# LikeLy-Journey/SegmenTron

Measured on AMD Instinct MI355X. Metric: images/sec fwd+bwd DeepLabv3+_xception65 @1025x2049, higher is better.
Workload: dtype bf16; 1 GPU; DeepLabv3+_xception65 train step (fwd + CE loss + bwd + SGD) @1025x2049, batch 2/GPU (BASELINE.json configs[2]); global_batch=2, bn=BN, parallelism=dp1, full_size=True

## Files before the change

### include/segmentron_hip.h

```cpp
#ifndef SEGMENTRON_HIP_H
#define SEGMENTRON_HIP_H
#ifdef __cplusplus
extern "C" {
#endif

const char* seg_last_error(void);
int seg_version(void);

int seg_conv_gemm_fwd(int dtype, const void* x, long ldx, int N, int Hi, int Wi, int C,
                      const void* w, int O, int KH, int KW, int stride, int pad, int dil,
                      int pro_mode, const float* pro_scale, const float* pro_shift,
                      const float* bias, void* y, long ldy, int Ho, int Wo, int out_H, int out_W,
                      int out_s, float* stat_partial, const void* ep_x, long ldep,
                      const float* ep_c0, const float* ep_c1, int tconv, void* stream);
int seg_conv_gemm_tiles_m(int N, int Ho, int Wo);

int seg_conv_gemm_wgrad(int dtype, const void* x, long ldx, int N, int Hi, int Wi, int C,
                        const void* dy, long lddy, int Ho, int Wo, int O, int KH, int KW,
                        int stride, int pad, int dil, int pro_mode, const float* pro_scale,
                        const float* pro_shift, float* partial, int splits, void* stream);
int seg_conv_gemm_stat_rows(int dtype, int N, int Ho, int Wo, int C, int O, int KH, int KW,
                            int stride, int pad, int dil, int tconv, int has_bias, int pro_mode);
int seg_conv_gemm_wgrad_splits(int dtype, int N, int Ho, int Wo, int C, int O, int KH, int KW,
                               int stride, int pad, int dil, int pro_mode);

int seg_dwconv3x3(int dtype, int mode, const void* x, long ldx, int N, int Hi, int Wi, int C,
                  const float* w9c, int w_layout, int stride, int dil, int pro_mode,
                  const float* pro_scale, const float* pro_shift, void* y, long ldy, int Ho, int Wo,
                  float* stat_partial, int grid_y, void* stream);
int seg_dwconv_grid_y(int dtype, int C, int N, int Ho, int Wo, int stride, int dil, int kind);
int seg_dwconv3x3_wgrad_finalize(const float* partial, int R, int C, float* dw_c9, void* stream);
int seg_dwconv3x3_wgrad(int dtype, const void* x, long ldx, int N, int Hi, int Wi, int C,
                        const void* dy, long lddy, int Ho, int Wo, int stride, int dil,
                        int pro_mode, const float* pro_scale, const float* pro_shift,
                        float* partial, int grid_y, void* stream);

int seg_dwconv3x3_bwd_fused(int dtype, const void* dy, long lddy, const void* x, long ldx, int N,
                            int H, int W, int C, const float* w9c, int w_layout, int dil,
                            int pro_mode, const float* pro_scale, const float* pro_shift, void* g,
                            long ldg, float* partial_w, float* partial_bn, int grid_y,
                            void* stream);
int seg_dwconv3x3_bwd_fused_add_ok(int dil);
int seg_dwconv3x3_bwd_fused_add(int dtype, const void* dy, long lddy, const void* x, long ldx, int N,
                                int H, int W, int C, const float* w9c, int w_layout, int pro_mode,
                                const float* pro_scale, const float* pro_shift, const void* res,
                                long ldr, void* g, long ldg, float* partial_w, float* partial_bn,
                                int grid_y, void* stream);

int seg_colsum(const float* in, long R, int L, double* out_d, float* out_f, double* ws,
               void* stream);
int seg_colsum_count(const float* in, long R, int L, double* out_d, double count, double* ws,
                     void* stream);
int seg_bn_finalize(const double* sums, double count, const double* count_dev,
                    const float* gamma, const float* beta, float eps, float momentum, float* running_mean, float* running_var,
                    float* mean, float* invstd, float* scale, float* shift, int C,
                    const float* mean_offset, void* stream);
int seg_bn_finalize_p(const float* partial, long R, double count, const float* gamma,
                      const float* beta, float eps, float momentum, float* running_mean,
                      float* running_var, float* mean, float* invstd, float* scale, float* shift,
                      int C, const float* mean_offset, double* ws, void* stream);
int seg_bn_finalize_small(int dtype, const void* y, long ldy, long M, int C, const float* gamma,
                          const float* beta, float eps, float momentum, float* running_mean,
                          float* running_var, float* mean, float* invstd, float* scale,
                          float* shift, const float* mean_offset, void* stream);
int seg_bn_moments_small(int dtype, const void* y, long ldy, long M, int C, double* moments,
                         void* stream);
int seg_bn_finalize_small_sync(void* p2p, int dtype, const void* y, long ldy, long M, int C,
                               const float* gamma, const float* beta, float eps, float momentum,
                               float* running_mean, float* running_var, float* mean, float* invstd,
                               float* scale, float* shift, const float* mean_offset,
// ... 197 lines not shown
```

### segmentron_amd/csrc/dwconv.hip

```cpp
#include "common.h"
#include "dwconv_tiled.h"
#include "dwconv_slide.h"
#include <cstdlib>
#include <type_traits>

namespace seg {

constexpr bool g_dw_row = true;

constexpr int DW_TW = 4;
constexpr int DW_THREADS = 256;
enum { MODE_FWD = 0, MODE_DGRAD = 1 };

struct DwArgs {
  const void* x;
  const float* w;
  void* y;
  const float* pro_scale;
  const float* pro_shift;
  float* stat_partial;
  long ldx, ldy;
  int N, Hi, Wi, C;
  int Ho, Wo;
  int stride, pad, dil;
// ... 527 lines not shown
                                           long ldx, int N, int H, int W, int C, const float* w9c,
                                           int w_layout, int pro_mode, const float* pro_scale,
                                           const float* pro_shift, const void* res, long ldr,
                                           void* g, long ldg, float* partial_w, float* partial_bn,
                                           int grid_y, void* stream) {
  using namespace seg;
  SEG_REQUIRE(dtype == DT_F32 || dtype == DT_BF16, "dwconv3x3_bwd_fused_add: bad dtype %d", dtype);
  const int tvec = dtype == DT_BF16 ? 8 : 4;
  SEG_REQUIRE(C % tvec == 0 && ldx % tvec == 0 && lddy % tvec == 0 && ldg % tvec == 0 &&
                  ldr % 4 == 0 && res != nullptr,
              "dwconv3x3_bwd_fused_add: C/ld must be multiples of %d, res non-null", tvec);
  SEG_REQUIRE(((pro_mode & PRO_AFFINE) == 0) || (pro_scale && pro_shift),
              "dwconv3x3_bwd_fused_add: affine prologue without scale/shift");
  SEG_REQUIRE(grid_y >= 1 && partial_w != nullptr, "dwconv3x3_bwd_fused_add: bad grid/partials");
  if (dw_slide_supported(1, 1, C))
    return launch_dw_slide_bwd(dtype, dy, lddy, x, ldx, N, H, W, C, w9c, w_layout, pro_mode,
                               pro_scale, pro_shift, g, ldg, partial_w, partial_bn, grid_y,
                               (hipStream_t)stream, res, ldr);
  return launch_dw_bwd_tiled(dtype, dy, lddy, x, ldx, N, H, W, C, w9c, w_layout, 1, pro_mode,
                             pro_scale, pro_shift, g, ldg, partial_w, partial_bn, grid_y,
                             (hipStream_t)stream, res, ldr);
}

extern "C" int seg_dwconv3x3_bwd_fused(int dtype, const void* dy, long lddy, const void* x,
                                       long ldx, int N, int H, int W, int C, const float* w9c,
                                       int w_layout, int dil, int pro_mode, const float* pro_scale,
                                       const float* pro_shift, void* g, long ldg,
                                       float* partial_w, float* partial_bn, int grid_y,
                                       void* stream) {
  using namespace seg;
  const int vec = 4;
  SEG_REQUIRE(dtype == DT_F32 || dtype == DT_BF16, "dwconv3x3_bwd_fused: bad dtype %d", dtype);
  SEG_REQUIRE(C % vec == 0 && ldx % vec == 0 && lddy % vec == 0 && ldg % vec == 0,
              "dwconv3x3_bwd_fused: C/ld must be multiples of %d", vec);
  SEG_REQUIRE(((pro_mode & PRO_AFFINE) == 0) || (pro_scale && pro_shift),
              "dwconv3x3_bwd_fused: affine prologue without scale/shift");
  SEG_REQUIRE(grid_y >= 1 && partial_w != nullptr, "dwconv3x3_bwd_fused: bad grid/partials");
  if (dw_slide_supported(1, dil, C))
    return launch_dw_slide_bwd(dtype, dy, lddy, x, ldx, N, H, W, C, w9c, w_layout, pro_mode,
                               pro_scale, pro_shift, g, ldg, partial_w, partial_bn, grid_y,
                               (hipStream_t)stream);
  if (dw_tiled_supported(1, dil)) {
    const int tvec = dtype == DT_BF16 ? 8 : 4;
    SEG_REQUIRE(C % tvec == 0 && ldx % tvec == 0 && lddy % tvec == 0 && ldg % tvec == 0,
                "dwconv3x3_bwd_fused: C/ld must be multiples of %d", tvec);
    return launch_dw_bwd_tiled(dtype, dy, lddy, x, ldx, N, H, W, C, w9c, w_layout, dil, pro_mode,
// ... 37 lines not shown
```

### segmentron_amd/csrc/dwconv_slide.h

```cpp
#pragma once
#include <hip/hip_runtime.h>

namespace seg {
bool dw_slide_supported(int stride, int dil, int C);
int dw_slide_rows(int C, int N, int H, int W);
int launch_dw_slide_fwd(int dtype, const void* x, long ldx, int N, int H, int W, int C,
                        const float* w, int w_layout, int pro_mode, const float* sc,
                        const float* sh, void* y, long ldy, float* stat_partial, int rows,
                        hipStream_t st);
int launch_dw_slide_bwd(int dtype, const void* dy, long lddy, const void* x, long ldx, int N, int H,
                        int W, int C, const float* w, int w_layout, int pro_mode, const float* sc,
                        const float* sh, void* g, long ldg, float* partial_w, float* partial_bn,
                        int rows, hipStream_t st, const void* res = nullptr, long ldr = 0);
}
```

### segmentron_amd/csrc/dwconv_slide.hip

```cpp
#include <type_traits>
#include "common.h"
#include "dwconv_slide.h"

namespace seg {

constexpr int SL_THREADS = 256, SL_CQ = 16, SL_WL = 16;
constexpr int SL_DEPTH_F = 2, SL_OCC_F = 4, SL_DEPTH_B = 2;
#define SL_SCHED_BARRIER() __builtin_amdgcn_sched_barrier(0)

struct DwSlideArgs {
  const void* x;
  const void* dy;
  const void* res;
  void* y;
  const float* w;
  int w_layout;
  const float* sc; const float* sh;
  float* partial;
  float* partial_bn;
  long ldx, lddy, ldy, ldr;
  int N, H, W, C, pro_mode, rs, nstrips, nwblk, ncblk;
};

struct SlBlock { int n, strip, wblk, cblk, prow; };
// ... 301 lines not shown
  if (a.partial != nullptr) {
    __shared__ float red[4][SL_CQ][8];
    float v[8] = {ssum.lo.x, ssum.lo.y, ssum.hi.x, ssum.hi.y, ssq.lo.x, ssq.lo.y, ssq.hi.x, ssq.hi.y};
#pragma unroll
    for (int i = 0; i < 8; ++i) {
      v[i] = t.live ? v[i] : 0.f;
      v[i] += __shfl_xor(v[i], 16, 64);
      v[i] += __shfl_xor(v[i], 32, 64);
    }
    if ((tid & 63) < SL_CQ) {
#pragma unroll
      for (int i = 0; i < 8; ++i) red[tid >> 6][cq][i] = v[i];
    }
    __syncthreads();
    if (tid < SL_CQ * 8) {
      const int q = tid >> 3, k = tid & 7;
      const float tot = red[0][q][k] + red[1][q][k] + red[2][q][k] + red[3][q][k];
      const int ch = (b.cblk * SL_CQ + q) * 4 + (k & 3);
      if (ch < a.C) a.partial[((long)b.prow * 2 + (k >> 2)) * a.C + ch] = tot;
    }
  }
}

template <typename T, int MODE, bool RES, bool XCHG>
__global__ __launch_bounds__(SL_THREADS, 2) void dwconv_slide_bwd_kernel(const DwSlideArgs a) {
  using IO = SlIO<T>;
  using raw_t = typename IO::raw_t;
  constexpr int ES = sizeof(T);
  const int tid = threadIdx.x, cq = tid & (SL_CQ - 1);
  const SlBlock b = sl_block(a);
  const SlThread t = sl_thread<ES>(a, b, a.lddy);
  const int r0 = t.r0, r1 = t.r1;

  Q4 wt[9], sc, sh;
  sc = sh = q4_zero();
  const long img = (long)b.n * a.H * a.W;
  const unsigned char* __restrict__ Db = reinterpret_cast<const unsigned char*>(a.dy) + img * a.lddy * ES;
  const unsigned char* __restrict__ Xb = reinterpret_cast<const unsigned char*>(a.x) + img * a.ldx * ES;
  const unsigned char* __restrict__ Rb =
      RES ? reinterpret_cast<const unsigned char*>(a.res) + img * a.ldr * ES : nullptr;
  unsigned char* __restrict__ Gb = reinterpret_cast<unsigned char*>(a.y) + img * a.ldy * ES;
  const long dpitch = (long)a.W * a.lddy * ES, xpitch = (long)a.W * a.ldx * ES;
  const long rpitch = (long)a.W * a.ldr * ES, gpitch = (long)a.W * a.ldy * ES;
  const unsigned rowbytes = (unsigned)dpitch;
  const unsigned xoff = (unsigned)((t.w * a.ldx + t.c) * ES), roff = (unsigned)((t.w * a.ldr + t.c) * ES);
  const unsigned goff = t.live ? (unsigned)((t.w * a.ldy + t.c) * ES) : 0xFFFFFFFFu;

  auto issue = [&](int r, raw_t (&raw)[3]) {
    const unsigned char* __restrict__ row = Db + (long)min(max(r, 0), t.rlast) * dpitch;
    if (XCHG) {
      raw[0] = sl_ld<raw_t>(row, t.off_0);
      raw[1] = sl_ld_edge<raw_t>(row, rowbytes, t.off_e);
    } else {
      raw[0] = sl_ld<raw_t>(row, t.off_0);
      raw[1] = sl_ld<raw_t>(row, t.off_m);
      raw[2] = sl_ld<raw_t>(row, t.off_p);
    }
  };
  auto issue_x = [&](int r, raw_t& xr, raw_t& rr) {
    const int rcl = min(r, r1 - 1);
    xr = sl_ld<raw_t>(Xb + (long)rcl * xpitch, xoff);
    if (RES) rr = sl_ld<raw_t>(Rb + (long)rcl * rpitch, roff);
  };
  auto commit = [&](int r, const raw_t (&raw)[3], Q4 (&row)[3], auto check) {
    constexpr bool CHECK = decltype(check)::value;
    const bool rv = !CHECK || (r >= 0 && r < a.H);
    raw_t r3[3];
    r3[1] = raw[0];
    if (XCHG) {
      sl_neighbours<raw_t>(t, raw, r3[0], r3[2]);
    } else {
      r3[0] = raw[1];
      r3[2] = raw[2];
    }
#pragma unroll
    for (int k = 0; k < 3; ++k) {
      row[k] = IO::unpack(r3[k]);
      if (CHECK && !rv) row[k] = q4_zero();
    }
  };
  Q4 accw[9], s1 = q4_zero(), s2 = q4_zero();
#pragma unroll
  for (int k = 0; k < 9; ++k) accw[k] = q4_zero();

  auto compute = [&](int ro, const raw_t& xraw, const raw_t& rraw, const Q4 (&ra)[3],
                     const Q4 (&rb)[3], const Q4 (&rcw)[3]) {
    const Q4 xr = IO::unpack(xraw);
    Q4 xa = xr;
    sl_act<MODE, false>(xa, sc, sh);
    Q4 g = q4_zero();
#pragma unroll
    for (int bq = 0; bq < 3; ++bq) { q4_fma(g, ra[bq], wt[8 - bq]); q4_fma(accw[8 - bq], ra[bq], xa); }
#pragma unroll
    for (int bq = 0; bq < 3; ++bq) { q4_fma(g, rb[bq], wt[5 - bq]); q4_fma(accw[5 - bq], rb[bq], xa); }
#pragma unroll
    for (int bq = 0; bq < 3; ++bq) { q4_fma(g, rcw[bq], wt[2 - bq]); q4_fma(accw[2 - bq], rcw[bq], xa); }
    if (MODE & PRO_RELU) {
      auto on = [&](float v) { return v > 0.f && (!(MODE & PRO_CLAMP6) || v < 6.f); };
      g.lo.x = on(xa.lo.x) ? g.lo.x : 0.f; g.lo.y = on(xa.lo.y) ? g.lo.y : 0.f;
      g.hi.x = on(xa.hi.x) ? g.hi.x : 0.f; g.hi.y = on(xa.hi.y) ? g.hi.y : 0.f;
    }
    if (RES) {
      const Q4 rr = IO::unpack(rraw);
      Q4 o;
      o.lo = g.lo + rr.lo;
      o.hi = g.hi + rr.hi;
      sl_st_row<raw_t>(Gb + (long)ro * gpitch, (unsigned)gpitch, goff, IO::pack(o));
    } else {
      sl_st_row<raw_t>(Gb + (long)ro * gpitch, (unsigned)gpitch, goff, IO::pack(g));
    }
    s1.lo += g.lo; s1.hi += g.hi;
    q4_fma(s2, g, xr);
  };

  constexpr int D = SL_DEPTH_B, U = (D % 3 == 0) ? D : 3 * D;
  Q4 win[3][3];
  raw_t ring[D][3], xring[D], rring[D];
#pragma unroll
  for (int j = 0; j < D; ++j) {
    issue(r0 - 1 + j, ring[j]);
    rring[j] = xring[j] = sl_ld<raw_t>(Xb + (long)min(r0 + j, r1 - 1) * xpitch, xoff);
    if (RES) rring[j] = sl_ld<raw_t>(Rb + (long)min(r0 + j, r1 - 1) * rpitch, roff);
  }
  sl_load_taps(a, t.c, wt);
  if (MODE & PRO_AFFINE) {
    const float4 s4 = *reinterpret_cast<const float4*>(a.sc + t.c);
    const float4 t4 = *reinterpret_cast<const float4*>(a.sh + t.c);
    sc.lo = (f32x2){s4.x, s4.y}; sc.hi = (f32x2){s4.z, s4.w};
    sh.lo = (f32x2){t4.x, t4.y}; sh.hi = (f32x2){t4.z, t4.w};
  }
#pragma unroll
  for (int kh = 0; kh < 3; ++kh) {
    if (!t.lm) wt[kh * 3 + 2] = q4_zero();
    if (!t.rm) wt[kh * 3] = q4_zero();
  }
  commit(r0 - 1, ring[0], win[0], std::true_type{});
  issue(r0 - 1 + D, ring[0]);
  commit(r0, ring[1 % D], win[1], std::false_type{});
  issue(r0 + D, ring[1 % D]);
  int ro = r0;
  for (; ro + U < r1; ro += U) {
#pragma unroll
    for (int k = 0; k < U; ++k) {
      commit(ro + k + 1, ring[(k + 2) % D], win[(k + 2) % 3], std::false_type{});
      issue(ro + k + 1 + D, ring[(k + 2) % D]);
      const raw_t xraw = xring[k % D], rraw = rring[k % D];
      issue_x(ro + k + D, xring[k % D], rring[k % D]);
      SL_SCHED_BARRIER();
      compute(ro + k, xraw, rraw, win[k % 3], win[(k + 1) % 3], win[(k + 2) % 3]);
      SL_SCHED_BARRIER();
    }
  }
#pragma unroll
  for (int k = 0; k < U; ++k) {
    if (ro + k < r1) {
      commit(ro + k + 1, ring[(k + 2) % D], win[(k + 2) % 3], std::true_type{});
      issue(ro + k + 1 + D, ring[(k + 2) % D]);
      const raw_t xraw = xring[k % D], rraw = rring[k % D];
      issue_x(ro + k + D, xring[k % D], rring[k % D]);
      compute(ro + k, xraw, rraw, win[k % 3], win[(k + 1) % 3], win[(k + 2) % 3]);
    }
  }

  float v[44];
#pragma unroll
  for (int k = 0; k < 9; ++k) {
    const int kw = k % 3;
    const bool keep = t.live && (kw != 2 || t.lm) && (kw != 0 || t.rm);
    v[k * 4] = keep ? accw[k].lo.x : 0.f; v[k * 4 + 1] = keep ? accw[k].lo.y : 0.f;
    v[k * 4 + 2] = keep ? accw[k].hi.x : 0.f; v[k * 4 + 3] = keep ? accw[k].hi.y : 0.f;
  }
  v[36] = s1.lo.x; v[37] = s1.lo.y; v[38] = s1.hi.x; v[39] = s1.hi.y;
  v[40] = s2.lo.x; v[41] = s2.lo.y; v[42] = s2.hi.x; v[43] = s2.hi.y;
#pragma unroll
  for (int i = 36; i < 44; ++i) v[i] = t.live ? v[i] : 0.f;
#pragma unroll
  for (int i = 0; i < 44; ++i) {
    v[i] += __shfl_xor(v[i], 16, 64);
    v[i] += __shfl_xor(v[i], 32, 64);
  }
  __shared__ float red[4][SL_CQ][44];
  if ((tid & 63) < SL_CQ) {
#pragma unroll
// ... 31 lines not shown
int dw_slide_rows(int C, int N, int H, int W) {
  DwSlideArgs a;
  slide_geom(a, N, H, W, C);
  return N * a.nstrips * a.nwblk;
}

static bool slide_exchange(const DwSlideArgs& a, int esize) {
  return (long)a.N * a.H * a.W * a.C * esize >= (30L << 20);
}
template <typename T>
static void slide_launch_fwd(const DwSlideArgs& a, dim3 grid, hipStream_t st) {
  const bool xc = slide_exchange(a, (int)sizeof(T));
  switch (a.pro_mode) {
#define SL_CASE(M)                                                                                  \
  case M:                                                                                           \
    if (xc) hipLaunchKernelGGL((dwconv_slide_fwd_kernel<T, M, true>), grid, dim3(SL_THREADS), 0, st, a);  \
    else hipLaunchKernelGGL((dwconv_slide_fwd_kernel<T, M, false>), grid, dim3(SL_THREADS), 0, st, a);    \
    break;
    SL_CASE(0) SL_CASE(1) SL_CASE(2) SL_CASE(3) SL_CASE(5) SL_CASE(7)
#undef SL_CASE
    default: break;
  }
}
template <typename T, bool RES>
static void slide_launch_bwd(const DwSlideArgs& a, dim3 grid, hipStream_t st) {
  const bool xc = slide_exchange(a, (int)sizeof(T));
  switch (a.pro_mode) {
#define SL_CASE(M)                                                                                       \
  case M:                                                                                                \
    if (xc) hipLaunchKernelGGL((dwconv_slide_bwd_kernel<T, M, RES, true>), grid, dim3(SL_THREADS), 0, st, a);  \
    else hipLaunchKernelGGL((dwconv_slide_bwd_kernel<T, M, RES, false>), grid, dim3(SL_THREADS), 0, st, a);    \
    break;
    SL_CASE(0) SL_CASE(1) SL_CASE(2) SL_CASE(3) SL_CASE(5) SL_CASE(7)
#undef SL_CASE
    default: break;
  }
}
static bool slide_mode_ok(int m) { return m == 0 || m == 1 || m == 2 || m == 3 || m == 5 || m == 7; }

int launch_dw_slide_fwd(int dtype, const void* x, long ldx, int N, int H, int W, int C,
                        const float* w, int w_layout, int pro_mode, const float* sc,
                        const float* sh, void* y, long ldy, float* stat_partial, int rows,
                        hipStream_t st) {
  DwSlideArgs a;
  a.x = x; a.dy = nullptr; a.res = nullptr; a.y = y; a.w = w; a.w_layout = w_layout;
  a.sc = sc; a.sh = sh; a.partial = stat_partial; a.partial_bn = nullptr;
  a.ldx = ldx; a.lddy = 0; a.ldy = ldy; a.ldr = 0;
  a.N = N; a.H = H; a.W = W; a.C = C; a.pro_mode = pro_mode;
  slide_geom(a, N, H, W, C);
  SEG_REQUIRE(slide_mode_ok(pro_mode), "dwconv (slide): unsupported prologue mode %d", pro_mode);
  SEG_REQUIRE(C % 4 == 0 && ldx % 4 == 0 && ldy % 4 == 0,
              "dwconv (slide): C/ldx/ldy must be multiples of 4");
  SEG_REQUIRE(stat_partial == nullptr || rows == N * a.nstrips * a.nwblk,
              "dwconv (slide): %d partial rows, the launch writes %d (seg_dwconv_grid_y)", rows,
              N * a.nstrips * a.nwblk);
  const dim3 grid((unsigned)((long)a.ncblk * a.nwblk * a.nstrips * N));
  if (dtype == DT_BF16) slide_launch_fwd<bf16_t>(a, grid, st);
  else slide_launch_fwd<float>(a, grid, st);
  return check_launch("dwconv3x3 (slide)");
}

int launch_dw_slide_bwd(int dtype, const void* dy, long lddy, const void* x, long ldx, int N, int H,
                        int W, int C, const float* w, int w_layout, int pro_mode, const float* sc,
                        const float* sh, void* g, long ldg, float* partial_w, float* partial_bn,
                        int rows, hipStream_t st, const void* res, long ldr) {
  DwSlideArgs a;
  a.x = x; a.dy = dy; a.res = res; a.y = g; a.w = w; a.w_layout = w_layout & 1;
  a.sc = sc; a.sh = sh; a.partial = partial_w; a.partial_bn = partial_bn;
  a.ldx = ldx; a.lddy = lddy; a.ldy = ldg; a.ldr = ldr;
  a.N = N; a.H = H; a.W = W; a.C = C; a.pro_mode = pro_mode;
  slide_geom(a, N, H, W, C);
  SEG_REQUIRE(slide_mode_ok(pro_mode), "dwconv bwd (slide): unsupported prologue mode %d", pro_mode);
  SEG_REQUIRE(C % 4 == 0 && ldx % 4 == 0 && lddy % 4 == 0 && ldg % 4 == 0 &&
                  (res == nullptr || ldr % 4 == 0),
              "dwconv bwd (slide): C/ldx/lddy/ldg/ldr must be multiples of 4");
  SEG_REQUIRE(rows == N * a.nstrips * a.nwblk,
              "dwconv bwd (slide): %d partial rows, the launch writes %d (seg_dwconv_grid_y)", rows,
              N * a.nstrips * a.nwblk);
  const dim3 grid((unsigned)((long)a.ncblk * a.nwblk * a.nstrips * N));
  if (dtype == DT_BF16) {
    if (res) slide_launch_bwd<bf16_t, true>(a, grid, st);
    else slide_launch_bwd<bf16_t, false>(a, grid, st);
  } else {
    if (res) slide_launch_bwd<float, true>(a, grid, st);
    else slide_launch_bwd<float, false>(a, grid, st);
  }
  return check_launch("dwconv3x3_bwd_fused (slide)");
}

}
```

### segmentron_amd/functional.py

```python
import contextlib
import dataclasses
import os
import weakref

import torch
import torch.distributed as dist
import torch.nn as nn

from . import hip_ops as K
from . import parallel
from .hip_ops import PRO_AFFINE, PRO_NONE, PRO_RELU


class BNState:
    __slots__ = ("gamma", "beta", "mean", "invstd", "scale", "shift", "count", "training", "group")

    def __init__(self, gamma, beta, mean, invstd, scale, shift, count, training, group=None):
        self.gamma, self.beta = gamma, beta
        self.mean, self.invstd, self.scale, self.shift = mean, invstd, scale, shift
        self.count, self.training, self.group = count, training, group


RELU, RELU6 = 1, 5

# ... 9 lines not shown
        mode = (PRO_AFFINE if self.bn is not None else PRO_NONE) | int(self.relu)
        if self.bn is None:
            return (mode, None, None)
        return (mode, self.bn.scale, self.bn.shift)

    @property
    def params(self):
        if self.bn is None:
            return None, None
        return self.bn.gamma, self.bn.beta

    def with_relu(self):
        return Act(self.t, self.bn, self.relu or True)

    @property
    def shape(self):
        return self.t.shape


_sync_group = parallel.sync_group


class GradFork:
    __slots__ = ("g",)

    def __init__(self):
        self.g = None

    def take(self):
        g, self.g = self.g, None
        return g


def uses_batch_stats(bn):
    return not getattr(bn, "frozen", False) and (bn.training or bn.running_mean is None)


def finish_bn(bn, partial, count, mean_offset=None, y=None):
    use_batch = uses_batch_stats(bn)
    if not use_batch:
        scale, shift = eval_affine(bn)
        invstd = mean = None
        if torch.is_grad_enabled():
            mean = bn.running_mean
            invstd = torch.rsqrt(bn.running_var + bn.eps)
        return BNState(bn.weight, bn.bias, mean, invstd, scale, shift, count, False)
    if count <= 1 and _sync_group(bn) is None:
        raise ValueError("Expected more than 1 value per channel when training, got count=%d"
                         % count)
    group = _sync_group(bn)
# ... 332 lines not shown
        else:
            dy_full = dy
        Cx = x.shape[-1]
        Ow = dy_full.shape[-1]
        dWp = K.conv_wgrad(x, dy_full, Ow, KH, KW, s.stride, s.pad, s.dil, s.pro)[:O]
        if KH == 1 and KW == 1 and Cx == Cw:
            dW = dWp.view(O, Cw, 1, 1)
        else:
            dW = dWp.view(O, KH, KW, Cx)[..., :Cw].permute(0, 3, 1, 2).contiguous()
        dbias = None
        if ctx.has_bias and s.drop_bias:
            dbias = torch.zeros(O, dtype=torch.float32, device=dy.device)
        elif ctx.has_bias:
            dbias = K.bn_bwd_reduce(dy_full, dy_full, (PRO_NONE, None, None))[:O].float()
        dx = dgamma = dbeta = None
        if ctx.needs_input_grad[0]:
            Op, dt = dy_full.shape[-1], x.dtype
            if KH == 1 and KW == 1 and Op == O and weight.dtype == torch.float32:
                wt = packed_pointwise(weight, True, dt)
            else:
                wt = cached_pack(weight, ("dgrad", Op, dt),
                                 lambda: pack_conv_weight_dgrad(weight, Op, dt))
            res = None
            if s.fork is not None and s.fork.g is not None:
                res = s.fork.take()
            if s.stride == 1 and res is not None and KH == 1 and KW == 1 and s.bn_in is None \
                    and not s.relu and Cw % K.vec_of(dt) == 0 and res.dtype == dt:
                g, _ = K.conv_gemm(dy_full, wt, Cw, 1, 1, 1, 0, 1,
                                   ep=(res, _const(Cw, x.device, 0.0), _const(Cw, x.device, -1.0)))
                res = None
            elif s.stride == 1:
                g, _ = K.conv_gemm(dy_full, wt, Cw, KH, KW, 1, s.dil * (KH - 1) - s.pad, s.dil)
            elif KH == 1 and KW == 1 and s.pad == 0:
                g, _ = K.conv_gemm(dy_full, wt, Cw, 1, 1, 1, 0, 1,
                                   scatter=(x.shape[1], x.shape[2], s.stride))
            else:
                wt = cached_pack(weight, ("tconv", Op, dt),
                                 lambda: pack_conv_weight_tconv(weight, Op, dt))
                g, _ = K.conv_gemm(dy_full, wt, Cw, KH, KW, s.stride, s.pad, s.dil,
                                   tconv_out_hw=(x.shape[1], x.shape[2]))
            dx, dgamma, dbeta = bn_input_backward(g, x, s.bn_in, s.relu, inplace=True)
            if res is not None:
                dx = dx + res
        elif s.fork is not None:
            s.fork.g = None
        return dx, dgamma, dbeta, dW, dbias, None

# ... 87 lines not shown
        ctx.save_for_backward(x, weight)
        return y

    @staticmethod
    def backward(ctx, dy):
        x, weight = ctx.saved_tensors
        s = ctx.spec
        C = weight.shape[0]
        if K.nhwc(dy)[4] % K.vec_of(dy.dtype) != 0:
            dy = dy.contiguous()
        dx = dgamma = dbeta = None
        tiled = K.dw_tiled(s.stride, s.dil)
        big = x.numel() * x.element_size() >= (40 << 20)
        strided = s.stride == 2 and s.dil == 1 and C % 4 == 0 and weight.dtype == torch.float32
        if ctx.needs_input_grad[0] and ((s.stride == 1 and (tiled or big or s.dil > 2)) or strided):
            bn = s.bn_in
            box = parallel.mailbox(bn.group) if (bn is not None and bn.group is not None) else None
            both = bn is not None and (strided or tiled) and \
                (bn.group is None or (box is not None and isinstance(bn.count, torch.Tensor)))
            if strided:
                g, dW, pb = K.dwconv_bwd_fused_s2(x, dy, weight.detach().contiguous(), s.pro,
                                                  want_bn=bn is not None, raw_dw=both)
            elif tiled:
                res = None
                if bn is None and s.fork is not None and s.fork.g is not None \
                        and K.dwconv_bwd_fused_add_ok(x, s.dil):
                    res = s.fork.take()
                    if res.dtype != x.dtype or tuple(res.shape) != tuple(x.shape):
                        s.fork.g, res = res, None
                g, dW, pb = K.dwconv_bwd_fused(x, dy, weight.detach(), s.dil, s.pro,
                                               want_bn=bn is not None, torch_layout=True,
                                               raw_dw=both, res=res)
            else:
                w9c = cached_pack(weight, "dw", lambda: pack_dw_weight(weight))
                g, dW9c, pb = K.dwconv_bwd_fused(x, dy, w9c, s.dil, s.pro, want_bn=bn is not None)
                dW = dW9c.t().reshape(C, 1, 3, 3).contiguous()
            if bn is None:
                dx = g
            else:
                if both and pb.shape[0] <= 1024 and bn.group is None:
                    dgamma, dbeta, c0, c1, dW = K.dw_bwd_finalize(pb, dW, bn.count, bn.mean,
                                                                  bn.invstd, bn.gamma)
                elif both and pb.shape[0] <= 1024:
                    dgamma, dbeta, c0, c1, dW = K.dw_bwd_finalize_sync(
                        box, pb, dW, bn.count, bn.mean, bn.invstd, bn.gamma,
                        parallel.grad_scale(bn.group))
                elif both:
                    dW = K.dw_wgrad_finalize(dW, C)
                    if bn.group is None:
                        dgamma, dbeta, c0, c1 = K.bn_bwd_finalize_p(pb, bn.count, bn.mean,
                                                                    bn.invstd, bn.gamma)
                    else:
                        dgamma, dbeta, c0, c1 = _sync_bwd_finalize(pb, bn)
                elif bn.group is None:
                    dgamma, dbeta, c0, c1 = K.bn_bwd_finalize_p(pb, bn.count, bn.mean, bn.invstd,
                                                                bn.gamma)
                else:
                    dgamma, dbeta, c0, c1 = _sync_bwd_finalize(pb, bn)
                if not bn.training:
                    c0 = c1 = None
                dx = K.bn_bwd_apply(g, x, (PRO_AFFINE, bn.scale, bn.shift), c0, c1, out=g)
        else:
            tiled = K.dw_tiled(s.stride, s.dil)
            if tiled:
                dW = K.dwconv_wgrad(x, dy, s.stride, s.dil, s.pro, torch_layout=True)
            else:
                dW9c = K.dwconv_wgrad(x, dy, s.stride, s.dil, s.pro)
                dW = dW9c.t().reshape(C, 1, 3, 3).contiguous()
            if ctx.needs_input_grad[0]:
                if tiled:
                    w = weight.detach()
                elif s.stride == 1:
                    w = cached_pack(weight, "dw_flip", lambda: pack_dw_weight(weight, True))
                else:
                    w = cached_pack(weight, "dw", lambda: pack_dw_weight(weight))
                g = K.dwconv_dgrad(dy, w, s.stride, s.dil, (x.shape[1], x.shape[2]))
                dx, dgamma, dbeta = bn_input_backward(g, x, s.bn_in, s.relu, inplace=True)
        if s.fork is not None and s.fork.g is not None and dx is not None:
            dx = dx + s.fork.take()
        return dx, dgamma, dbeta, dW, None


class ApplySpec:
    def __init__(self, a, r=None, chan_mul=None, post_relu=False, out=None, elem_mul=None,
                 fork=None):
        self.elem_mul = elem_mul
        self.fork = fork
        self.bn_x, self.relu_x, self.pro_x = a.bn, a.relu, a.pro
        if r is not None:
            self.bn_r, self.relu_r, self.pro_r = r.bn, r.relu, r.pro
        else:
            self.bn_r, self.relu_r, self.pro_r = None, False, None
        self.chan_mul, self.post_relu, self.out = chan_mul, post_relu, out


class _ApplyFn(torch.autograd.Function):

    @staticmethod
    def forward(ctx, x, gx, bx, r, gr, br, spec):
        y = K.bn_apply(x, spec.pro_x, r, spec.pro_r, spec.chan_mul, spec.post_relu, spec.out,
                       spec.elem_mul)
# ... 424 lines not shown
        dgamma = _dot(dout, raw) if ctx.needs_input_grad[1] else None
        do = _scaled(dout, g32)
        dx = torch.empty_like(x)
        for n in range(N):
            a, xn, don = atts[n], x[n].reshape(P, C).contiguous(), do[n].reshape(P, C)
            de = K.row_softmax_bwd(a, K.gemm_tn(don, xn), C, torch.float32, sign=-1.0)
            sym = (de + de.t()).to(dt)
            g1 = K.gemm_nt(don, a.t().contiguous()).view(1, H, W, C)
            g2 = K.gemm_nt(xn, sym).view(1, H, W, C)
            K.bn_apply(g1, None, g2, None, out=dx[n:n + 1])
        dx = K.bn_apply(dx, None, dout, None)
        return dx, dgamma


def position_attention(q, k, v, x, gamma):
    return _PAMFn.apply(q, k, v, x, gamma)


def channel_attention(x, gamma):
    return _CAMFn.apply(x, gamma)


_NO_FOLD = os.environ.get("SEG_NO_FOLD") == "1"


class _GroupNormFn(torch.autograd.Function):

    @staticmethod
    def forward(ctx, y, weight, bias, groups, eps, out):
        N, H, W, C = y.shape
        mean_rstd, coef = K.gn_fwd_finalize(K.gn_moments(y), H * W, groups, weight, bias, eps)
        ctx.save_for_backward(y, weight, mean_rstd)
        ctx.groups, ctx.has_bias = groups, bias is not None
        return K.gn_affine(y, None, coef, out=out)

    @staticmethod
    def backward(ctx, dz):
        y, weight, mean_rstd = ctx.saved_tensors
        N, H, W, C = y.shape
        if dz.dtype != y.dtype:
            dz = dz.to(y.dtype)
        if not _sum_n_operand_ok(dz, K.vec_of(y.dtype)):
            dz = dz.contiguous()
        coef, contrib = K.gn_bwd_finalize(K.gn_moments(dz, y), H * W, ctx.groups, mean_rstd, weight)
        dx = K.gn_affine(dz, y, coef) if ctx.needs_input_grad[0] else None
        dw = db = None
# ... 140 lines not shown
```

### segmentron_amd/hip_ops.py

```python
import torch

from ._lib import LIB

PRO_NONE, PRO_RELU, PRO_AFFINE, PRO_AFFINE_RELU = 0, 1, 2, 3
_DT = {torch.float32: 0, torch.bfloat16: 1}


def vec_of(dtype):
    return 8 if dtype == torch.bfloat16 else 4


_raw_stream = getattr(torch._C, "_cuda_getCurrentRawStream", None)


def _stream():
    if _raw_stream is not None:
        return _raw_stream(torch.cuda.current_device())
    return torch.cuda.current_stream().cuda_stream


def _p(t):
    return 0 if t is None else t.data_ptr()


# ... 223 lines not shown
    C = mean.numel()
    out = torch.empty((4, C), dtype=torch.float32, device=mean.device)
    dW = torch.empty((C, 1, 3, 3), dtype=torch.float32, device=mean.device)
    LIB.call("seg_dw_bwd_finalize", _p(pb), pb.shape[0], float(count), _p(mean), _p(invstd),
             _p(gamma), _p(out[0]), _p(out[1]), _p(out[2]), _p(out[3]), _p(pw), pw.shape[0],
             _p(dW), C, _stream())
    return out[0], out[1], out[2], out[3], dW


def dw_bwd_finalize_sync(box, pb, pw, count_dev, mean, invstd, gamma, grad_scale):
    C = mean.numel()
    out = torch.empty((4, C), dtype=torch.float32, device=mean.device)
    dW = torch.empty((C, 1, 3, 3), dtype=torch.float32, device=mean.device)
    LIB.call("seg_dw_bwd_finalize_sync", box.handle, _p(pb), pb.shape[0], _p(count_dev), _p(mean),
             _p(invstd), _p(gamma), _p(out[0]), _p(out[1]), _p(out[2]), _p(out[3]), _p(pw),
             pw.shape[0], _p(dW), C, float(grad_scale), _stream())
    return out[0], out[1], out[2], out[3], dW


def dwconv_bwd_fused_add_ok(x, dil):
    return bool(LIB.query("seg_dwconv3x3_bwd_fused_add_ok", int(dil)))


def dwconv_bwd_fused(x, dy, w, dil, pro=None, want_bn=False, torch_layout=False, raw_dw=False,
                     res=None, out=None):
    N, H, W, C, ldx = nhwc(x)
    lddy = nhwc(dy)[4]
    mode, ps, pt = _pro(pro)
    g, ldg = _dw_grad_out(out, N, H, W, C, x)
    tiled = dw_tiled(1, dil)
    layout = 1 if w.dim() == 4 else 0
    if layout and not tiled:
        raise ValueError("depthwise strip kernels need tap-major [9, C] weights")
    gy = LIB.query("seg_dwconv_grid_y", _DT[x.dtype], C, N, H, W, 1, dil, 1)
    pw = torch.empty((gy, 9 * C), dtype=torch.float32, device=x.device)
    pb = torch.empty((gy, 2 * C), dtype=torch.float32, device=x.device) if want_bn else None
    if res is not None:
        assert dil == 1 and tuple(res.shape) == (N, H, W, C) and res.dtype == x.dtype
        LIB.call("seg_dwconv3x3_bwd_fused_add", _DT[x.dtype], _p(dy), lddy, _p(x), ldx, N, H, W,
                 C, _p(w), layout, mode, _p(ps), _p(pt), _p(res), nhwc(res)[4], _p(g), ldg, _p(pw),
                 _p(pb), gy, _stream())
    else:
        LIB.call("seg_dwconv3x3_bwd_fused", _DT[x.dtype], _p(dy), lddy, _p(x), ldx, N, H, W, C,
                 _p(w), layout, dil, mode, _p(ps), _p(pt), _p(g), ldg, _p(pw), _p(pb), gy, _stream())
    if raw_dw:
        return g, pw, pb
    if torch_layout:
        dW = torch.empty((C, 1, 3, 3), dtype=torch.float32, device=x.device)
        LIB.call("seg_dwconv3x3_wgrad_finalize", _p(pw), gy, C, _p(dW), _stream())
        return g, dW, pb
    return g, colsum(pw, f64=False).view(9, C), pb


def dwconv_bwd_fused_s2(x, dy, w, pro=None, want_bn=False, raw_dw=False, out=None):
    N, H, W, C, ldx = nhwc(x)
    Nd, Ho, Wo, Cd, lddy = nhwc(dy)
    assert (Nd, Ho, Wo, Cd) == (N, (H + 1) // 2, (W + 1) // 2, C) and tuple(w.shape) == (C, 1, 3, 3)
    mode, ps, pt = _pro(pro)
    g, ldg = _dw_grad_out(out, N, H, W, C, x)
    gy = LIB.query("seg_dwconv3x3_s2_grid_y", C, N, H, W)
# ... 713 lines not shown
```

### segmentron_amd/models/backbones/xception.py

```python
import torch
import torch.nn as nn

from ... import functional as F
from ...config import cfg
from ...modules import SeparableConv2d
from .build import BACKBONE_REGISTRY

__all__ = ["Xception65", "XceptionBlock", "xception65"]


class XceptionBlock(nn.Module):

    def __init__(self, channel_list, stride=1, dilation=1, skip_connection_type="conv",
                 relu_first=True, low_feat=False, norm_layer=nn.BatchNorm2d):
        super().__init__()
        assert len(channel_list) == 4
        if skip_connection_type not in ("conv", "sum", "none"):
            raise ValueError("Unsupported skip connection type.")
        self.skip_connection_type = skip_connection_type
        self.relu_first = relu_first
        self.low_feat = low_feat
        c = channel_list
        if skip_connection_type == "conv":
            self.conv = nn.Conv2d(c[0], c[3], 1, stride=stride, bias=False)
            self.bn = norm_layer(c[3])
        self.sep_conv1 = SeparableConv2d(c[0], c[1], dilation=dilation, relu_first=relu_first,
                                         norm_layer=norm_layer)
        self.sep_conv2 = SeparableConv2d(c[1], c[2], dilation=dilation, relu_first=relu_first,
                                         norm_layer=norm_layer)
        self.sep_conv3 = SeparableConv2d(c[2], c[3], dilation=dilation, relu_first=relu_first,
                                         stride=stride, norm_layer=norm_layer)
        self.last_inp_channels = c[3]

    def forward(self, inputs):
        fork = None
        if (self.skip_connection_type == "sum" and self.relu_first and inputs.bn is None
                and not inputs.relu and torch.is_grad_enabled() and inputs.t.requires_grad):
            fork = F.GradFork()
        skip_in = inputs
        if self.skip_connection_type == "conv":
            t = F.fork(inputs.t, 2)
            inputs, skip_in = F.Act(t[0], inputs.bn, inputs.relu), F.Act(t[1], inputs.bn, inputs.relu)
        sc1 = self.sep_conv1(inputs, fork=fork) if fork is not None else self.sep_conv1(inputs)
        sc2 = self.sep_conv2(sc1)
        low = sc2
        if self.low_feat:
            t = F.fork(sc2.t, 2)
            sc2, low = F.Act(t[0], sc2.bn, sc2.relu), F.Act(t[1], sc2.bn, sc2.relu)
        residual = self.sep_conv3(sc2)
        if self.skip_connection_type == "conv":
            shortcut = F.conv_bn(skip_in, self.conv, self.bn)
            outputs = F.Act(F.materialize(residual, residual=shortcut))
        elif self.skip_connection_type == "sum":
            outputs = F.Act(F.materialize(residual, residual=inputs, fork=fork))
        else:
            outputs = residual
        return (outputs, low) if self.low_feat else outputs


class Xception65(nn.Module):

    def __init__(self, norm_layer=nn.BatchNorm2d):
        super().__init__()
        os_ = cfg.MODEL.OUTPUT_STRIDE
        if os_ == 32:
            b3_stride, mid_dil, exit_dil, exit_stride = 2, 1, (1, 1), 2
        elif os_ == 16:
            b3_stride, mid_dil, exit_dil, exit_stride = 2, 1, (1, 2), 1
        elif os_ == 8:
            b3_stride, mid_dil, exit_dil, exit_stride = 1, 2, (2, 4), 1
        else:
            raise NotImplementedError
        self.conv1 = nn.Conv2d(3, 32, 3, stride=2, padding=1, bias=False)
        self.bn1 = norm_layer(32)
# ... 40 lines not shown
```

Measured before the change: 89.68 images/sec.

## Fuse strided 1x1 skip-conv input gradient into depthwise backward kernel

In Xception conv-skip blocks, the skip branch's 1x1 conv dgrad now computes its gradient at the compact (possibly stride-2) resolution and parks it in a GradFork. The first separable conv's depthwise backward kernel then adds it in, either upsampling the stride-2 residual by parity-selecting even positions or adding it before the BN/ReLU mask. This removes the separate strided scatter or dgrad of the shortcut and the extra elementwise add of two full-size gradient tensors. It adds new kernel template variants and more complex autograd bookkeeping, and it is limited to blocks with fewer than 256 output channels when BN comes first.

```diff
diff --git a/include/segmentron_hip.h b/include/segmentron_hip.h
--- a/include/segmentron_hip.h
+++ b/include/segmentron_hip.h
@@ -46,6 +46,13 @@
                                 const float* pro_scale, const float* pro_shift, const void* res,
                                 long ldr, void* g, long ldg, float* partial_w, float* partial_bn,
                                 int grid_y, void* stream);
+int seg_dwconv3x3_bwd_fused_skip_ok(int dtype, int C, int res_stride, int before_mask, int dil,
+                                    int pro_mode);
+int seg_dwconv3x3_bwd_fused_skip(int dtype, const void* dy, long lddy, const void* x, long ldx, int N,
+                                 int H, int W, int C, const float* w9c, int w_layout, int pro_mode,
+                                 const float* pro_scale, const float* pro_shift, const void* res,
+                                 long ldr, int res_stride, int before_mask, void* g, long ldg,
+                                 float* partial_w, float* partial_bn, int grid_y, void* stream);
 
 int seg_colsum(const float* in, long R, int L, double* out_d, float* out_f, double* ws,
                void* stream);
diff --git a/segmentron_amd/csrc/dwconv.hip b/segmentron_amd/csrc/dwconv.hip
--- a/segmentron_amd/csrc/dwconv.hip
+++ b/segmentron_amd/csrc/dwconv.hip
@@ -573,6 +573,41 @@
                              (hipStream_t)stream, res, ldr);
 }
 
+extern "C" int seg_dwconv3x3_bwd_fused_skip_ok(int dtype, int C, int res_stride, int before_mask,
+                                               int dil, int pro_mode) {
+  using namespace seg;
+  if ((dtype != DT_F32 && dtype != DT_BF16) || dil != 1 || (res_stride != 1 && res_stride != 2))
+    return 0;
+  if (res_stride == 1 && before_mask) return 0;
+  const int rm = res_stride == 1 ? SL_RES_FULL : (before_mask ? SL_RES_C2_PRE : SL_RES_C2);
+  return dw_slide_res_ok(rm, pro_mode, C) ? 1 : 0;
+}
+
+extern "C" int seg_dwconv3x3_bwd_fused_skip(int dtype, const void* dy, long lddy, const void* x,
+                                            long ldx, int N, int H, int W, int C, const float* w9c,
+                                            int w_layout, int pro_mode, const float* pro_scale,
+                                            const float* pro_shift, const void* res, long ldr,
+                                            int res_stride, int before_mask, void* g, long ldg,
+                                            float* partial_w, float* partial_bn, int grid_y,
+                                            void* stream) {
+  using namespace seg;
+  SEG_REQUIRE(seg_dwconv3x3_bwd_fused_skip_ok(dtype, C, res_stride, before_mask, 1, pro_mode),
+              "dwconv3x3_bwd_fused_skip: dtype %d C %d res_stride %d before_mask %d prologue %d is "
+              "not served", dtype, C, res_stride, before_mask, pro_mode);
+  SEG_REQUIRE(ldx % 4 == 0 && lddy % 4 == 0 && ldg % 4 == 0 && ldr % 4 == 0 && ldr >= C &&
+                  res != nullptr,
+              "dwconv3x3_bwd_fused_skip: pitches must be multiples of 4, res non-null");
+  SEG_REQUIRE(((pro_mode & PRO_AFFINE) == 0) || (pro_scale && pro_shift),
+              "dwconv3x3_bwd_fused_skip: affine prologue without scale/shift");
+  SEG_REQUIRE(grid_y >= 1 && partial_w != nullptr, "dwconv3x3_bwd_fused_skip: bad grid/partials");
+  SEG_REQUIRE(!before_mask || partial_bn != nullptr,
+              "dwconv3x3_bwd_fused_skip: before_mask without BatchNorm-backward partials");
+  const int rm = res_stride == 1 ? SL_RES_FULL : (before_mask ? SL_RES_C2_PRE : SL_RES_C2);
+  return launch_dw_slide_bwd(dtype, dy, lddy, x, ldx, N, H, W, C, w9c, w_layout, pro_mode,
+                             pro_scale, pro_shift, g, ldg, partial_w, partial_bn, grid_y,
+                             (hipStream_t)stream, res, ldr, rm);
+}
+
 extern "C" int seg_dwconv3x3_bwd_fused(int dtype, const void* dy, long lddy, const void* x,
                                        long ldx, int N, int H, int W, int C, const float* w9c,
                                        int w_layout, int dil, int pro_mode, const float* pro_scale,
diff --git a/segmentron_amd/csrc/dwconv_slide.h b/segmentron_amd/csrc/dwconv_slide.h
--- a/segmentron_amd/csrc/dwconv_slide.h
+++ b/segmentron_amd/csrc/dwconv_slide.h
@@ -2,6 +2,7 @@
 #include <hip/hip_runtime.h>
 
 namespace seg {
+enum SlRes { SL_RES_NONE = 0, SL_RES_FULL = 1, SL_RES_C2 = 2, SL_RES_C2_PRE = 3 };
 bool dw_slide_supported(int stride, int dil, int C);
 int dw_slide_rows(int C, int N, int H, int W);
 int launch_dw_slide_fwd(int dtype, const void* x, long ldx, int N, int H, int W, int C,
@@ -11,5 +12,7 @@
 int launch_dw_slide_bwd(int dtype, const void* dy, long lddy, const void* x, long ldx, int N, int H,
                         int W, int C, const float* w, int w_layout, int pro_mode, const float* sc,
                         const float* sh, void* g, long ldg, float* partial_w, float* partial_bn,
-                        int rows, hipStream_t st, const void* res = nullptr, long ldr = 0);
+                        int rows, hipStream_t st, const void* res = nullptr, long ldr = 0,
+                        int res_mode = -1);
+bool dw_slide_res_ok(int res_mode, int pro_mode, int C);
 }
diff --git a/segmentron_amd/csrc/dwconv_slide.hip b/segmentron_amd/csrc/dwconv_slide.hip
--- a/segmentron_amd/csrc/dwconv_slide.hip
+++ b/segmentron_amd/csrc/dwconv_slide.hip
@@ -347,14 +347,16 @@
   }
 }
 
-template <typename T, int MODE, bool RES, bool XCHG>
+template <typename T, int MODE, int RM, bool XCHG>
 __global__ __launch_bounds__(SL_THREADS, 2) void dwconv_slide_bwd_kernel(const DwSlideArgs a) {
   using IO = SlIO<T>;
   using raw_t = typename IO::raw_t;
   constexpr int ES = sizeof(T);
+  constexpr bool RES = RM != SL_RES_NONE, C2 = RM == SL_RES_C2 || RM == SL_RES_C2_PRE;
   const int tid = threadIdx.x, cq = tid & (SL_CQ - 1);
   const SlBlock b = sl_block(a);
   const SlThread t = sl_thread<ES>(a, b, a.lddy);
+  const int Hc = (a.H + 1) >> 1, Wc = (a.W + 1) >> 1;
   const int r0 = t.r0, r1 = t.r1;
 
   Q4 wt[9], sc, sh;
@@ -363,12 +365,17 @@
   const unsigned char* __restrict__ Db = reinterpret_cast<const unsigned char*>(a.dy) + img * a.lddy * ES;
   const unsigned char* __restrict__ Xb = reinterpret_cast<const unsigned char*>(a.x) + img * a.ldx * ES;
   const unsigned char* __restrict__ Rb =
-      RES ? reinterpret_cast<const unsigned char*>(a.res) + img * a.ldr * ES : nullptr;
+      RES ? reinterpret_cast<const unsigned char*>(a.res) + (C2 ? (long)b.n * Hc * Wc : img) * a.ldr * ES
+          : nullptr;
   unsigned char* __restrict__ Gb = reinterpret_cast<unsigned char*>(a.y) + img * a.ldy * ES;
   const long dpitch = (long)a.W * a.lddy * ES, xpitch = (long)a.W * a.ldx * ES;
-  const long rpitch = (long)a.W * a.ldr * ES, gpitch = (long)a.W * a.ldy * ES;
+  const long rpitch = (long)(C2 ? Wc : a.W) * a.ldr * ES, gpitch = (long)a.W * a.ldy * ES;
   const unsigned rowbytes = (unsigned)dpitch;
-  const unsigned xoff = (unsigned)((t.w * a.ldx + t.c) * ES), roff = (unsigned)((t.w * a.ldr + t.c) * ES);
+  const unsigned xoff = (unsigned)((t.w * a.ldx + t.c) * ES);
+  const unsigned roff = (unsigned)(((C2 ? t.w >> 1 : t.w) * a.ldr + t.c) * ES);
+  const bool weven = (t.w & 1) == 0;
+  const bool rsel0 = weven && (t.r0 & 1) == 0, rsel1 = weven && (t.r0 & 1) != 0;
+  const raw_t rzero = IO::pack(q4_zero());
   const unsigned goff = t.live ? (unsigned)((t.w * a.ldy + t.c) * ES) : 0xFFFFFFFFu;
 
   auto issue = [&](int r, raw_t (&raw)[3]) {
@@ -385,7 +392,7 @@
   auto issue_x = [&](int r, raw_t& xr, raw_t& rr) {
     const int rcl = min(r, r1 - 1);
     xr = sl_ld<raw_t>(Xb + (long)rcl * xpitch, xoff);
-    if (RES) rr = sl_ld<raw_t>(Rb + (long)rcl * rpitch, roff);
+    if (RES) rr = sl_ld<raw_t>(Rb + (long)(C2 ? rcl >> 1 : rcl) * rpitch, roff);
   };
   auto commit = [&](int r, const raw_t (&raw)[3], Q4 (&row)[3], auto check) {
     constexpr bool CHECK = decltype(check)::value;
@@ -408,9 +415,15 @@
 #pragma unroll
   for (int k = 0; k < 9; ++k) accw[k] = q4_zero();
 
-  auto compute = [&](int ro, const raw_t& xraw, const raw_t& rraw, const Q4 (&ra)[3],
+  auto compute = [&](int ro, int kpar, const raw_t& xraw, const raw_t& rraw, const Q4 (&ra)[3],
                      const Q4 (&rb)[3], const Q4 (&rcw)[3]) {
     const Q4 xr = IO::unpack(xraw);
+    Q4 rr = q4_zero();
+    if (RES) {
+      raw_t rz = rraw;
+      if (C2) rz = sl_sel(kpar ? rsel1 : rsel0, rraw, rzero);
+      rr = IO::unpack(rz);
+    }
     Q4 xa = xr;
     sl_act<MODE, false>(xa, sc, sh);
     Q4 g = q4_zero();
@@ -420,13 +433,16 @@
     for (int bq = 0; bq < 3; ++bq) { q4_fma(g, rb[bq], wt[5 - bq]); q4_fma(accw[5 - bq], rb[bq], xa); }
 #pragma unroll
     for (int bq = 0; bq < 3; ++bq) { q4_fma(g, rcw[bq], wt[2 - bq]); q4_fma(accw[2 - bq], rcw[bq], xa); }
+    if (RM == SL_RES_C2_PRE) {
+      g.lo = g.lo + rr.lo;
+      g.hi = g.hi + rr.hi;
+    }
     if (MODE & PRO_RELU) {
       auto on = [&](float v) { return v > 0.f && (!(MODE & PRO_CLAMP6) || v < 6.f); };
       g.lo.x = on(xa.lo.x) ? g.lo.x : 0.f; g.lo.y = on(xa.lo.y) ? g.lo.y : 0.f;
       g.hi.x = on(xa.hi.x) ? g.hi.x : 0.f; g.hi.y = on(xa.hi.y) ? g.hi.y : 0.f;
     }
-    if (RES) {
-      const Q4 rr = IO::unpack(rraw);
+    if (RES && RM != SL_RES_C2_PRE) {
       Q4 o;
       o.lo = g.lo + rr.lo;
       o.hi = g.hi + rr.hi;
@@ -439,13 +455,14 @@
   };
 
   constexpr int D = SL_DEPTH_B, U = (D % 3 == 0) ? D : 3 * D;
+  static_assert(U % 2 == 0, "the compact residual's row parity follows the unrolled step");
   Q4 win[3][3];
   raw_t ring[D][3], xring[D], rring[D];
 #pragma unroll
   for (int j = 0; j < D; ++j) {
     issue(r0 - 1 + j, ring[j]);
     rring[j] = xring[j] = sl_ld<raw_t>(Xb + (long)min(r0 + j, r1 - 1) * xpitch, xoff);
-    if (RES) rring[j] = sl_ld<raw_t>(Rb + (long)min(r0 + j, r1 - 1) * rpitch, roff);
+    if (RES) rring[j] = sl_ld<raw_t>(Rb + (long)(C2 ? min(r0 + j, r1 - 1) >> 1 : min(r0 + j, r1 - 1)) * rpitch, roff);
   }
   sl_load_taps(a, t.c, wt);
   if (MODE & PRO_AFFINE) {
@@ -472,7 +489,7 @@
       const raw_t xraw = xring[k % D], rraw = rring[k % D];
       issue_x(ro + k + D, xring[k % D], rring[k % D]);
       SL_SCHED_BARRIER();
-      compute(ro + k, xraw, rraw, win[k % 3], win[(k + 1) % 3], win[(k + 2) % 3]);
+      compute(ro + k, k & 1, xraw, rraw, win[k % 3], win[(k + 1) % 3], win[(k + 2) % 3]);
       SL_SCHED_BARRIER();
     }
   }
@@ -483,7 +500,7 @@
       issue(ro + k + 1 + D, ring[(k + 2) % D]);
       const raw_t xraw = xring[k % D], rraw = rring[k % D];
       issue_x(ro + k + D, xring[k % D], rring[k % D]);
-      compute(ro + k, xraw, rraw, win[k % 3], win[(k + 1) % 3], win[(k + 2) % 3]);
+      compute(ro + k, k & 1, xraw, rraw, win[k % 3], win[(k + 1) % 3], win[(k + 2) % 3]);
     }
   }
 
@@ -561,21 +578,38 @@
     default: break;
   }
 }
-template <typename T, bool RES>
+template <typename T, int RM>
 static void slide_launch_bwd(const DwSlideArgs& a, dim3 grid, hipStream_t st) {
   const bool xc = slide_exchange(a, (int)sizeof(T));
   switch (a.pro_mode) {
 #define SL_CASE(M)                                                                                       \
   case M:                                                                                                \
-    if (xc) hipLaunchKernelGGL((dwconv_slide_bwd_kernel<T, M, RES, true>), grid, dim3(SL_THREADS), 0, st, a);  \
-    else hipLaunchKernelGGL((dwconv_slide_bwd_kernel<T, M, RES, false>), grid, dim3(SL_THREADS), 0, st, a);    \
+    if (xc) hipLaunchKernelGGL((dwconv_slide_bwd_kernel<T, M, RM, true>), grid, dim3(SL_THREADS), 0, st, a);  \
+    else hipLaunchKernelGGL((dwconv_slide_bwd_kernel<T, M, RM, false>), grid, dim3(SL_THREADS), 0, st, a);    \
     break;
     SL_CASE(0) SL_CASE(1) SL_CASE(2) SL_CASE(3) SL_CASE(5) SL_CASE(7)
 #undef SL_CASE
     default: break;
   }
 }
+template <typename T, int RM, int M>
+static void slide_launch_bwd_one(const DwSlideArgs& a, dim3 grid, hipStream_t st) {
+  if (slide_exchange(a, (int)sizeof(T)))
+    hipLaunchKernelGGL((dwconv_slide_bwd_kernel<T, M, RM, true>), grid, dim3(SL_THREADS), 0, st, a);
+  else
+    hipLaunchKernelGGL((dwconv_slide_bwd_kernel<T, M, RM, false>), grid, dim3(SL_THREADS), 0, st, a);
+}
 static bool slide_mode_ok(int m) { return m == 0 || m == 1 || m == 2 || m == 3 || m == 5 || m == 7; }
+
+bool dw_slide_res_ok(int res_mode, int pro_mode, int C) {
+  if (!dw_slide_supported(1, 1, C) || !slide_mode_ok(pro_mode)) return false;
+  switch (res_mode) {
+    case SL_RES_NONE: case SL_RES_FULL: return true;
+    case SL_RES_C2: return pro_mode == PRO_NONE || pro_mode == PRO_RELU;
+    case SL_RES_C2_PRE: return pro_mode == (PRO_AFFINE | PRO_RELU);
+    default: return false;
+  }
+}
 
 int launch_dw_slide_fwd(int dtype, const void* x, long ldx, int N, int H, int W, int C,
                         const float* w, int w_layout, int pro_mode, const float* sc,
@@ -602,7 +636,11 @@
 int launch_dw_slide_bwd(int dtype, const void* dy, long lddy, const void* x, long ldx, int N, int H,
                         int W, int C, const float* w, int w_layout, int pro_mode, const float* sc,
                         const float* sh, void* g, long ldg, float* partial_w, float* partial_bn,
-                        int rows, hipStream_t st, const void* res, long ldr) {
+                        int rows, hipStream_t st, const void* res, long ldr, int res_mode) {
+  if (res_mode < 0) res_mode = res ? SL_RES_FULL : SL_RES_NONE;
+  SEG_REQUIRE((res != nullptr) == (res_mode != SL_RES_NONE) && dw_slide_res_ok(res_mode, pro_mode, C),
+              "dwconv bwd (slide): residual mode %d is not served with prologue mode %d", res_mode,
+              pro_mode);
   DwSlideArgs a;
   a.x = x; a.dy = dy; a.res = res; a.y = g; a.w = w; a.w_layout = w_layout & 1;
   a.sc = sc; a.sh = sh; a.partial = partial_w; a.partial_bn = partial_bn;
@@ -617,13 +655,24 @@
               "dwconv bwd (slide): %d partial rows, the launch writes %d (seg_dwconv_grid_y)", rows,
               N * a.nstrips * a.nwblk);
   const dim3 grid((unsigned)((long)a.ncblk * a.nwblk * a.nstrips * N));
+#define SL_RES_DISPATCH(T)                                                                        \
+  switch (res_mode) {                                                                             \
+    case SL_RES_FULL: slide_launch_bwd<T, SL_RES_FULL>(a, grid, st); break;                       \
+    case SL_RES_C2:                                                                               \
+      if (pro_mode == PRO_RELU) slide_launch_bwd_one<T, SL_RES_C2, PRO_RELU>(a, grid, st);        \
+      else slide_launch_bwd_one<T, SL_RES_C2, PRO_NONE>(a, grid, st);                             \
+      break;                                                                                      \
+    case SL_RES_C2_PRE:                                                                           \
+      slide_launch_bwd_one<T, SL_RES_C2_PRE, PRO_AFFINE | PRO_RELU>(a, grid, st);                 \
+      break;                                                                                      \
+    default: slide_launch_bwd<T, SL_RES_NONE>(a, grid, st); break;                                \
+  }
   if (dtype == DT_BF16) {
-    if (res) slide_launch_bwd<bf16_t, true>(a, grid, st);
-    else slide_launch_bwd<bf16_t, false>(a, grid, st);
+    SL_RES_DISPATCH(bf16_t)
   } else {
-    if (res) slide_launch_bwd<float, true>(a, grid, st);
-    else slide_launch_bwd<float, false>(a, grid, st);
-  }
+    SL_RES_DISPATCH(float)
+  }
+#undef SL_RES_DISPATCH
   return check_launch("dwconv3x3_bwd_fused (slide)");
 }
 
diff --git a/segmentron_amd/functional.py b/segmentron_amd/functional.py
--- a/segmentron_amd/functional.py
+++ b/segmentron_amd/functional.py
@@ -55,10 +55,11 @@
 
 
 class GradFork:
-    __slots__ = ("g",)
-
-    def __init__(self):
+    __slots__ = ("g", "skip", "before", "closed")
+
+    def __init__(self, skip=0, before=False):
         self.g = None
+        self.skip, self.before, self.closed = skip, before, False
 
     def take(self):
         g, self.g = self.g, None
@@ -437,7 +438,13 @@
                 wt = cached_pack(weight, ("dgrad", Op, dt),
                                  lambda: pack_conv_weight_dgrad(weight, Op, dt))
             res = None
-            if s.fork is not None and s.fork.g is not None:
+            if s.fork is not None and s.fork.skip:
+                f = s.fork
+                if not f.closed and _SKIP_HANDOFF and f.skip == s.stride and KH == 1 and KW == 1 \
+                        and s.pad == 0:
+                    f.g, _ = K.conv_gemm(dy_full, wt, Cw, 1, 1, 1, 0, 1)
+                    return None, None, None, dW, dbias, None
+            elif s.fork is not None and s.fork.g is not None:
                 res = s.fork.take()
             if s.stride == 1 and res is not None and KH == 1 and KW == 1 and s.bn_in is None \
                     and not s.relu and Cw % K.vec_of(dt) == 0 and res.dtype == dt:
@@ -571,15 +578,26 @@
                 g, dW, pb = K.dwconv_bwd_fused_s2(x, dy, weight.detach().contiguous(), s.pro,
                                                   want_bn=bn is not None, raw_dw=both)
             elif tiled:
-                res = None
-                if bn is None and s.fork is not None and s.fork.g is not None \
+                res = skip = None
+                if s.fork is not None and s.fork.skip:
+                    f = s.fork
+                    if f.g is None:
+                        f.closed = True
+                    else:
+                        if f.before != (bn is not None) or not K.dwconv_bwd_fused_skip_ok(
+                                x.dtype, C, f.skip, f.before, s.dil, s.pro[0]):
+                            raise RuntimeError("conv-skip hand-off: no kernel takes the parked "
+                                               "gradient (stride %d, before=%s, prologue %d)"
+                                               % (f.skip, f.before, s.pro[0]))
+                        res, skip = f.take(), (f.skip, f.before)
+                elif bn is None and s.fork is not None and s.fork.g is not None \
                         and K.dwconv_bwd_fused_add_ok(x, s.dil):
                     res = s.fork.take()
                     if res.dtype != x.dtype or tuple(res.shape) != tuple(x.shape):
                         s.fork.g, res = res, None
                 g, dW, pb = K.dwconv_bwd_fused(x, dy, weight.detach(), s.dil, s.pro,
                                                want_bn=bn is not None, torch_layout=True,
-                                               raw_dw=both, res=res)
+                                               raw_dw=both, res=res, skip=skip)
             else:
                 w9c = cached_pack(weight, "dw", lambda: pack_dw_weight(weight))
                 g, dW9c, pb = K.dwconv_bwd_fused(x, dy, w9c, s.dil, s.pro, want_bn=bn is not None)
@@ -625,7 +643,11 @@
                     w = cached_pack(weight, "dw", lambda: pack_dw_weight(weight))
                 g = K.dwconv_dgrad(dy, w, s.stride, s.dil, (x.shape[1], x.shape[2]))
                 dx, dgamma, dbeta = bn_input_backward(g, x, s.bn_in, s.relu, inplace=True)
-        if s.fork is not None and s.fork.g is not None and dx is not None:
+        if s.fork is not None and s.fork.skip:
+            if s.fork.g is not None:
+                raise RuntimeError("conv-skip hand-off: the parked gradient was not taken")
+            s.fork.closed = True
+        elif s.fork is not None and s.fork.g is not None and dx is not None:
             dx = dx + s.fork.take()
         return dx, dgamma, dbeta, dW, None
 
@@ -1096,6 +1118,31 @@
 
 
 _NO_FOLD = os.environ.get("SEG_NO_FOLD") == "1"
+_SKIP_HANDOFF = os.environ.get("SEG_NO_SKIP_HANDOFF") != "1"
+
+
+def skip_fork(inputs, conv, dw_conv):
+    t = inputs.t
+    if not (_SKIP_HANDOFF and torch.is_grad_enabled() and t.requires_grad):
+        return None
+    stride = conv.stride[0]
+    if conv.kernel_size != (1, 1) or conv.padding[0] != 0 or stride not in (1, 2) \
+            or conv.stride[1] != stride or conv.bias is not None:
+        return None
+    if dw_conv.stride[0] != 1 or dw_conv.dilation[0] != 1 or t.dim() != 4:
+        return None
+    bn = inputs.bn
+    if bn is None and not inputs.relu:
+        before, mode = False, PRO_RELU
+    elif bn is not None and inputs.relu is True and bn.group is None:
+        before, mode = True, PRO_AFFINE | PRO_RELU
+        if conv.out_channels >= 256:
+            return None
+    else:
+        return None
+    if not K.dwconv_bwd_fused_skip_ok(t.dtype, t.shape[-1], stride, before, 1, mode):
+        return None
+    return GradFork(skip=stride, before=before)
 
 
 class _GroupNormFn(torch.autograd.Function):
diff --git a/segmentron_amd/hip_ops.py b/segmentron_amd/hip_ops.py
--- a/segmentron_amd/hip_ops.py
+++ b/segmentron_amd/hip_ops.py
@@ -269,8 +269,13 @@
     return bool(LIB.query("seg_dwconv3x3_bwd_fused_add_ok", int(dil)))
 
 
+def dwconv_bwd_fused_skip_ok(dtype, C, res_stride, before_mask, dil, pro_mode):
+    return bool(LIB.query("seg_dwconv3x3_bwd_fused_skip_ok", _DT[dtype], int(C), int(res_stride),
+                          int(bool(before_mask)), int(dil), int(pro_mode)))
+
+
 def dwconv_bwd_fused(x, dy, w, dil, pro=None, want_bn=False, torch_layout=False, raw_dw=False,
-                     res=None, out=None):
+                     res=None, out=None, skip=None):
     N, H, W, C, ldx = nhwc(x)
     lddy = nhwc(dy)[4]
     mode, ps, pt = _pro(pro)
@@ -282,7 +287,14 @@
     gy = LIB.query("seg_dwconv_grid_y", _DT[x.dtype], C, N, H, W, 1, dil, 1)
     pw = torch.empty((gy, 9 * C), dtype=torch.float32, device=x.device)
     pb = torch.empty((gy, 2 * C), dtype=torch.float32, device=x.device) if want_bn else None
-    if res is not None:
+    if skip is not None:
+        rs, before = skip
+        assert res is not None and res.dtype == x.dtype and dil == 1 and (want_bn or not before)
+        assert tuple(res.shape) == (N, (H + rs - 1) // rs, (W + rs - 1) // rs, C)
+        LIB.call("seg_dwconv3x3_bwd_fused_skip", _DT[x.dtype], _p(dy), lddy, _p(x), ldx, N, H, W,
+                 C, _p(w), layout, mode, _p(ps), _p(pt), _p(res), nhwc(res)[4], int(rs),
+                 int(bool(before)), _p(g), ldg, _p(pw), _p(pb), gy, _stream())
+    elif res is not None:
         assert dil == 1 and tuple(res.shape) == (N, H, W, C) and res.dtype == x.dtype
         LIB.call("seg_dwconv3x3_bwd_fused_add", _DT[x.dtype], _p(dy), lddy, _p(x), ldx, N, H, W,
                  C, _p(w), layout, mode, _p(ps), _p(pt), _p(res), nhwc(res)[4], _p(g), ldg, _p(pw),
diff --git a/segmentron_amd/models/backbones/xception.py b/segmentron_amd/models/backbones/xception.py
--- a/segmentron_amd/models/backbones/xception.py
+++ b/segmentron_amd/models/backbones/xception.py
@@ -39,6 +39,8 @@
             fork = F.GradFork()
         skip_in = inputs
         if self.skip_connection_type == "conv":
+            if self.relu_first:
+                fork = F.skip_fork(inputs, self.conv, self.sep_conv1.block.depthwise)
             t = F.fork(inputs.t, 2)
             inputs, skip_in = F.Act(t[0], inputs.bn, inputs.relu), F.Act(t[1], inputs.bn, inputs.relu)
         sc1 = self.sep_conv1(inputs, fork=fork) if fork is not None else self.sep_conv1(inputs)
@@ -49,7 +51,7 @@
             sc2, low = F.Act(t[0], sc2.bn, sc2.relu), F.Act(t[1], sc2.bn, sc2.relu)
         residual = self.sep_conv3(sc2)
         if self.skip_connection_type == "conv":
-            shortcut = F.conv_bn(skip_in, self.conv, self.bn)
+            shortcut = F.conv_bn(skip_in, self.conv, self.bn, fork=fork)
             outputs = F.Act(F.materialize(residual, residual=shortcut))
         elif self.skip_connection_type == "sum":
             outputs = F.Act(F.materialize(residual, residual=inputs, fork=fork))
```

Measured after the change: 90.10 images/sec, median of 6. About the same (+0.5%).
